# SiftScience/kafka-assigner

Measured on NVIDIA H100. Metric: partition-replica assignments/sec, higher is better.
Workload: dtype int32

## Files before the change

### kafka_assigner_b200/csrc/kassign.cu

```cuda
#include "kassign_stage.cuh"
#include "kassign_order.cuh"
#include "kassign_json.cuh"
#include "kassign_score.cuh"
#include "kassign_waves.cuh"
#include "kassign_waves_json.cuh"
#include "kassign_usage.cuh"

#include <algorithm>
#include <climits>
#include <cmath>
#include <cstdio>
#include <cstdlib>
#include <cstring>
#include <map>
#include <new>
#include <string>
#include <unordered_map>
#include <vector>

#include "../../include/kassign.h"

namespace {

constexpr int KA_SM_COUNT_FALLBACK = 132;
constexpr size_t KA_SMEM_BUDGET = 200 * 1024;
constexpr uint32_t KA_LUT_SMEM_MAX_RANGE = 32768;
constexpr uint32_t KA_LUT_GLOBAL_MAX_RANGE = 1u << 25;

struct DevBuf {
    void* p = nullptr;
    size_t cap = 0;
    cudaError_t reserve(size_t bytes) {
        if (bytes <= cap) return cudaSuccess;
        if (p) cudaFree(p);
        p = nullptr;
        cap = 0;
        size_t want = bytes + bytes / 8 + 256;
        cudaError_t e = cudaMalloc(&p, want);
        if (e == cudaSuccess) cap = want;
        return e;
    }
    void release() {
        if (p) cudaFree(p);
        p = nullptr;
        cap = 0;
    }
    template <typename T> T* as() const { return reinterpret_cast<T*>(p); }
};

constexpr int KA_MAX_BLOCKS = 8;
constexpr int KA_MAX_CHAIN_BLOCKS = 16;
constexpr int KA_MAX_CHAIN_EVENTS = KA_MAX_BLOCKS * KA_MAX_CHAIN_BLOCKS;
constexpr int KA_MAX_JSON_FRAGS = 256;
constexpr int KA_MAX_CANDIDATES = 128;
static_assert(KA_MAX_CANDIDATES <= KA_JSON_MAX_SEGS, "a fleet's documents are built in one segmented JSON pass");
constexpr int64_t KA_JSON_FRAG_ROWS = 1 << 18;

struct HostPinned {
    int err_topic;
    int spin_flag;
    int4 tstatus;
};

struct Plan {
    int a_blob_bytes;
    int a_warps, a_load_bytes, a_slab_bytes, a_cnt_bytes, a_load_kind;
    int a_levels;
    int lv_owner_bytes, lv_last_bytes, lv_p_bytes;
    size_t a_smem;
    int rec_kind, rec_bytes;
    int b_gctr;
    int b_ring_log2;
    int b_threads;
    size_t b_smem;
};

struct StageDesc {
    int topic_base = 0, T = 0;
    int64_t Q = 0;
    const int32_t* d_hash = nullptr;
    const int64_t* d_part_off = nullptr;
    const int64_t* d_rep_off = nullptr;
    int P = 0, RF = 0;
    const int32_t* d_cur = nullptr;
    int desired_rf = -1, S = 1, Pmax = 0;
    int64_t capmax = 0;
    int64_t q0 = 0;
    int blk = 0;
    Plan pl;
};

struct RunScratch {
    DevBuf rec, perm, ntl, lend, loff, lvl_end, tstatus, flags;
    cudaError_t reserve(size_t rec_bytes, size_t q, size_t T, size_t nloff, bool levels, size_t nflags) {
        const struct { DevBuf* b; size_t bytes; } want[] = {
            {&rec, rec_bytes}, {&perm, levels ? q * 2 : 0}, {&lend, levels ? q * 4 : 0}, {&lvl_end, levels ? q * 4 : 0},
            {&ntl, levels ? T * 4 : 0}, {&loff, levels ? nloff * 4 : 0}, {&tstatus, T * sizeof(int4)}, {&flags, nflags * 4},
        };
        for (const auto& w : want)
            if (cudaError_t e = w.b->reserve(w.bytes)) return e;
        return cudaSuccess;
    }
    void release() {
        for (DevBuf* b : {&rec, &perm, &ntl, &lend, &loff, &lvl_end, &tstatus, &flags}) b->release();
    }
};

}

struct ka_ctx {
    int device = 0;
    int sm_count = KA_SM_COUNT_FALLBACK;
    cudaStream_t stream = nullptr;
    cudaStream_t aux = nullptr;
    cudaStream_t sb1 = nullptr;
    cudaStream_t sj = nullptr;
    KaBrokers br{};
    std::vector<int32_t> broker_id;
    DevBuf d_blob, d_glut, d_broker_id, d_ctr8;
    std::unordered_map<int32_t, std::vector<int32_t>> parked;
    int64_t launches = 0;
    DevBuf d_hash, d_part_off, d_rep_off, d_cur, d_out, d_out_len;
    RunScratch run;
    DevBuf d_json, d_names, d_name_off, d_part_id, d_json_rowlen, d_json_blocksum, d_json_state;
    DevBuf d_json_seg;
    DevBuf d_batch_tab, d_batch_ctr;
    RunScratch batch_run;
    DevBuf d_score_w, d_score_sum, d_score_brk, d_score_off;
    DevBuf d_wv_nrecv, d_wv_wave, d_wv_tmp, d_wv_rec, d_wv_cnt, d_wv_state, d_wv_log, d_wv_sum, d_wv_meta;
    DevBuf d_wv_send, d_wv_slog, d_wv_ssum;
    DevBuf d_wv_perm, d_wv_hist, d_wv_doc;
    DevBuf d_wv_part, d_wv_jump;
    DevBuf d_wv_back, d_wv_bscr;
    DevBuf d_us_id, d_us_base, d_us_cap, d_us_before, d_us_ev, d_us_hist, d_us_out, d_us_meta;
    HostPinned* h_pin = nullptr;
    unsigned long long* h_frag = nullptr;
    cudaEvent_t ev[6] = {};
    cudaEvent_t ev_pipe[KA_MAX_BLOCKS][5] = {};
    cudaEvent_t ev_chain[KA_MAX_BLOCKS][4] = {};
    cudaEvent_t ev_in = nullptr, ev_stage[KA_MAX_BLOCKS] = {}, ev_chain_in = nullptr, ev_b1[KA_MAX_CHAIN_EVENTS] = {};
    cudaEvent_t ev_b2[KA_MAX_CHAIN_EVENTS] = {}, ev_emit_done = nullptr;
    cudaEvent_t ev_json_in[KA_MAX_JSON_FRAGS] = {}, ev_json_scan[KA_MAX_JSON_FRAGS] = {}, ev_out_done = nullptr;
    bool timing = false;
    float last_ms[8] = {};
    bool ev_valid = false;
    int last_stages = 1;
    int chain_used = 0;
    bool slot_timed[2] = {false, false};
    int32_t order_plan[8] = {};
    int32_t stage_plan[8] = {};
    bool staged = false;
    StageDesc staged_block;
    int topic_base = 0;
    bool last_was_staged = false;
    cudaStream_t last_stream = nullptr;
    bool pending_status = false;
    ka_status last{};
};

namespace {

#define KA_CUDA(call)                                                                              \
    do {                                                                                           \
        cudaError_t _e = (call);                                                                   \
        if (_e != cudaSuccess) {                                                                   \
            std::fprintf(stderr, "[kassign] CUDA error %s at %s:%d: %s\n", cudaGetErrorName(_e), __FILE__, __LINE__, \
                         cudaGetErrorString(_e));                                                  \
            return KA_ERR_CUDA;                                                                    \
        }                                                                                          \
    } while (0)

int set_status(ka_status* st, int code, int topic = -1, int part = -1, int a = 0, int b = 0) {
    if (st) {
        st->code = code;
        st->topic_index = topic;
        st->partition = part;
        st->a = a;
        st->b = b;
    }
    return code;
}

int failed(ka_status* st, int rc) {
    if (st && st->code != rc) set_status(st, rc);
    return rc;
}

inline size_t align16(size_t v) { return (v + 15) & ~size_t(15); }

template <typename F>
void for_each_event(ka_ctx* c, F f) {
    const struct { cudaEvent_t* e; size_t n; bool timed; } pools[] = {
        {c->ev, sizeof(c->ev) / sizeof(cudaEvent_t), true},
        {&c->ev_pipe[0][0], sizeof(c->ev_pipe) / sizeof(cudaEvent_t), true},
        {&c->ev_chain[0][0], sizeof(c->ev_chain) / sizeof(cudaEvent_t), true},
        {&c->ev_in, 1, false},
        {c->ev_stage, KA_MAX_BLOCKS, false},
        {&c->ev_chain_in, 1, false},
        {c->ev_b1, KA_MAX_CHAIN_EVENTS, false},
        {c->ev_b2, KA_MAX_CHAIN_EVENTS, false},
        {&c->ev_emit_done, 1, false},
        {c->ev_json_in, KA_MAX_JSON_FRAGS, false},
        {c->ev_json_scan, KA_MAX_JSON_FRAGS, false},
        {&c->ev_out_done, 1, false},
    };
    for (const auto& p : pools)
        for (size_t i = 0; i < p.n; ++i) f(p.e[i], p.timed);
}

int park_counters(ka_ctx* c) {
    if (c->br.N == 0 || !c->d_ctr8.p) return KA_OK;
    std::vector<int32_t> h((size_t)c->br.N * KA_MAX_SLOTS);
    KA_CUDA(cudaMemcpy(h.data(), c->d_ctr8.p, h.size() * 4, cudaMemcpyDeviceToHost));
    for (int i = 0; i < c->br.N; ++i) {
        const int32_t* row = h.data() + (size_t)i * KA_MAX_SLOTS;
        bool nz = false;
        for (int r = 0; r < KA_MAX_SLOTS; ++r) nz |= row[r] != 0;
        if (nz) c->parked[c->broker_id[i]] = std::vector<int32_t>(row, row + KA_MAX_SLOTS);
        else c->parked.erase(c->broker_id[i]);
    }
    return KA_OK;
}

int check_brokers(int N, const int32_t* broker_id, const int32_t* broker_rack) {
    if (N < 0 || (N > 0 && (!broker_id || !broker_rack))) return KA_ERR_BAD_ARG;
    if (N > 65535) return KA_ERR_LIMIT;
    for (int i = 0; i < N; ++i) {
        if (i > 0 && broker_id[i] <= broker_id[i - 1]) return KA_ERR_BAD_ARG;
        if (broker_rack[i] < 0 || broker_rack[i] >= 65535) return KA_ERR_BAD_ARG;
    }
    return KA_OK;
}

struct BrokerTable {
    int lut_mode = KA_LUT_SMEM, min_id = 0, lut_off = 0;
    uint32_t range = 0;
    std::vector<uint16_t> blob, glut;
    int blob_bytes() const { return (int)(blob.size() * 2); }
    KaBrokers device(int N, const uint16_t* d_blob, const uint16_t* d_glut, const int32_t* d_broker_id) const {
        return KaBrokers{N, lut_mode, lut_off, blob_bytes(), min_id, range, d_blob, d_glut, d_broker_id};
    }
};

BrokerTable broker_table(int N, const int32_t* broker_id, const int32_t* broker_rack) {
    BrokerTable t;
    t.min_id = N > 0 ? broker_id[0] : 0;
    const uint64_t range64 = N > 0 ? (uint64_t)((int64_t)broker_id[N - 1] - (int64_t)broker_id[0]) + 1 : 0;
    const size_t npad = align16((size_t)std::max(N, 1) * 2) / 2;
    std::vector<uint16_t> rackc(std::max(N, 1), 0);
    {
// ... 121 lines not shown
    d.T = t1 - t0;
    d.blk = blk;
    d.q0 = (int64_t)t0 * sh.P;
    d.Q = ragged ? sh.Q : (int64_t)d.T * sh.P;
    d.d_hash = sh.d_hash + t0;
    d.d_part_off = sh.d_part_off;
    d.d_rep_off = sh.d_rep_off;
    d.P = sh.P;
    d.RF = sh.RF;
    d.d_cur = sh.d_cur + d.q0 * sh.RF;
    d.desired_rf = sh.desired_rf;
    d.S = sh.S;
    d.Pmax = sh.Pmax;
    d.capmax = sh.capmax;
    return make_plan(N, blob_bytes, d.Q, d.S, d.Pmax, d.capmax, ragged, d.pl, st);
}

int reserve_scratch(ka_ctx* c, const StageDesc* ds, int K) {
    const StageDesc& e = ds[K - 1];
    const size_t q = (size_t)std::max<int64_t>(e.q0 + e.Q, 1);
    const size_t T = (size_t)std::max(e.topic_base + e.T, 1);
    KA_CUDA(c->run.reserve(q * ds[0].pl.rec_bytes + 256, q, T, T + K + 1, ds[0].pl.a_levels, 16));
    return KA_OK;
}

int reserve_io(ka_ctx* c, Shape& sh, bool ragged) {
    KA_CUDA(c->d_hash.reserve((size_t)std::max(sh.T, 1) * 4));
    if (ragged) {
        KA_CUDA(c->d_part_off.reserve((size_t)(sh.T + 1) * 8));
        KA_CUDA(c->d_rep_off.reserve((size_t)(sh.Q + 1) * 8));
    }
    KA_CUDA(c->d_cur.reserve((size_t)std::max<int64_t>(sh.R, 1) * 4));
    KA_CUDA(c->d_out.reserve((size_t)std::max<int64_t>(sh.Q, 1) * sh.S * 4));
    KA_CUDA(c->d_out_len.reserve((size_t)std::max<int64_t>(sh.Q, 1) * 4));
    sh.d_hash = c->d_hash.as<int32_t>();
    sh.d_cur = c->d_cur.as<int32_t>();
    if (ragged) {
        sh.d_part_off = c->d_part_off.as<int64_t>();
        sh.d_rep_off = c->d_rep_off.as<int64_t>();
    }
    return KA_OK;
}

int reset_flags(ka_ctx* c, cudaStream_t s) {
    c->h_pin->err_topic = -1;
    c->h_pin->spin_flag = -1;
    c->chain_used = 0;
    c->slot_timed[0] = c->slot_timed[1] = false;
    KA_CUDA(cudaMemsetAsync(c->run.flags.p, 0xFF, 2 * sizeof(int), s));
    return KA_OK;
}

template <typename LoadT, bool LEVELS, int SM, bool CAND>
cudaError_t launch_stage_t(ka_ctx* c, cudaStream_t s, const KaSolveParams& p, const Plan& pl, int T, int ncand, int* grid_x) {
    auto kern = ka_sticky_spread_kernel<LoadT, LEVELS, SM, CAND>;
    const int threads = pl.a_warps * 32;
    cudaError_t e = allow_smem(kern, pl.a_smem);
    if (e != cudaSuccess) return e;
    int occ = 1;
    e = cudaOccupancyMaxActiveBlocksPerMultiprocessor(&occ, kern, threads, pl.a_smem);
    if (e != cudaSuccess) return e;
    int grid = (T + pl.a_warps - 1) / pl.a_warps;
    grid = std::min(grid, std::max(1, std::max(1, occ) * c->sm_count / std::max(ncand, 1)));
    *grid_x = grid;
    kern<<<dim3(grid, std::max(ncand, 1)), threads, pl.a_smem, s>>>(p, pl.a_load_bytes, pl.a_slab_bytes, pl.a_cnt_bytes, pl.lv_owner_bytes,
                                                                 pl.lv_last_bytes, pl.lv_p_bytes);
    return cudaGetLastError();
}

template <typename LoadT, bool LEVELS, bool CAND>
cudaError_t launch_stage(ka_ctx* c, cudaStream_t s, const KaSolveParams& p, const Plan& pl, int T, int ncand, int* grid_x) {
    return p.S <= 3 ? launch_stage_t<LoadT, LEVELS, 3, CAND>(c, s, p, pl, T, ncand, grid_x)
                    : launch_stage_t<LoadT, LEVELS, 8, CAND>(c, s, p, pl, T, ncand, grid_x);
}

void reset_plans(ka_ctx* c) {
    for (int32_t& v : c->order_plan) v = 0;
    for (int32_t& v : c->stage_plan) v = 0;
}

template <bool CAND>
int launch_stage_plan(ka_ctx* c, cudaStream_t s, const KaSolveParams& p, const Plan& pl, int T, int ncand, int lut_mask) {
    cudaError_t e;
    int grid_x = 0;
    if (!pl.a_levels) e = launch_stage<uint8_t, false, CAND>(c, s, p, pl, T, ncand, &grid_x);
    else if (pl.a_load_kind == 0) e = launch_stage<uint8_t, true, CAND>(c, s, p, pl, T, ncand, &grid_x);
    else e = launch_stage<uint16_t, true, CAND>(c, s, p, pl, T, ncand, &grid_x);
    KA_CUDA(e);
    c->launches++;
    int32_t* r = c->stage_plan;
    r[0] = pl.a_load_kind == 0 ? 1 : 2;
    r[1] = pl.a_levels;
    r[2] = p.S <= 3 ? 3 : 8;
    r[3] = ncand;
    r[4] = pl.a_warps;
    r[5] = grid_x;
    r[6] = lut_mask;
    r[7]++;
    return KA_OK;
}

KaSolveParams stage_params(const StageDesc& d) {
    KaSolveParams p{};
    p.T = d.T;
    p.topic_base = d.topic_base;
    p.topic_hash = d.d_hash;
    p.part_off = d.d_part_off;
    p.P = d.P;
    p.rep_off = d.d_rep_off;
    p.RF = d.RF;
    p.cur = d.d_cur;
    p.desired_rf = d.desired_rf;
    p.S = d.S;
    p.Pmax = d.Pmax;
    p.blob_space = d.pl.a_blob_bytes;
    p.rec_kind = d.pl.rec_kind;
    p.chunk_w = d.pl.b_threads;
    return p;
}

int enq_stage(ka_ctx* c, cudaStream_t s, const StageDesc& d, cudaEvent_t a_done, cudaEvent_t done = nullptr) {
    const Plan& pl = d.pl;
    RunScratch& r = c->run;
    if (d.T > 0) {
        KaSolveParams p = stage_params(d);
        p.br = c->br;
        p.out.rec = r.rec.as<unsigned char>() + (size_t)d.q0 * pl.rec_bytes;
        p.out.perm = pl.a_levels ? r.perm.as<uint16_t>() + d.q0 : nullptr;
        p.out.ntl = pl.a_levels ? r.ntl.as<int32_t>() + d.topic_base : nullptr;
        p.out.lend = pl.a_levels ? r.lend.as<uint32_t>() + d.q0 : nullptr;
        p.out.tstatus = r.tstatus.as<int4>();
        p.out.err_topic = r.flags.as<unsigned>();
        const int rc = launch_stage_plan<false>(c, s, p, pl, d.T, 0, 1 << c->br.lut_mode);
        if (rc != KA_OK) return rc;
    }
    const bool tables = pl.a_levels && d.T > 0;
    if (done && !tables) KA_CUDA(cudaEventRecord(done, s));
    if (c->timing) KA_CUDA(cudaEventRecord(a_done, s));
    if (tables) {
        int32_t* ntl = r.ntl.as<int32_t>() + d.topic_base;
        int32_t* loff = r.loff.as<int32_t>() + d.topic_base + d.blk;
        ka_level_scan_kernel<<<1, 1024, 0, s>>>(ntl, d.T, loff);
        KA_CUDA(cudaGetLastError());
        ka_level_fill_kernel<<<(d.T + 7) / 8, 256, 0, s>>>(ntl, loff, r.lend.as<uint32_t>() + d.q0, d.d_part_off, d.P, d.T, d.T, d.Q,
                                                            r.lvl_end.as<uint32_t>() + d.q0);
        KA_CUDA(cudaGetLastError());
        c->launches += 2;
        if (done) KA_CUDA(cudaEventRecord(done, s));
    }
    return KA_OK;
}

template <int KIND, int MAXNT, bool CAND, bool GCTR, bool SINGLE, bool WARP1, bool FULL>
cudaError_t launch_order_t(cudaStream_t s, const KaOrderParams& o, const Plan& pl, int ncand, bool behind) {
    auto kern = ka_order_levels_kernel<KIND, GCTR, MAXNT, SINGLE, WARP1, FULL, CAND>;
    cudaError_t e = allow_smem(kern, pl.b_smem);
    if (e != cudaSuccess) return e;
    cudaLaunchAttribute attr{};
    attr.id = cudaLaunchAttributeProgrammaticStreamSerialization;
    attr.val.programmaticStreamSerializationAllowed = 1;
    cudaLaunchConfig_t cfg{};
    cfg.gridDim = dim3(CAND ? ncand : 1);
    cfg.blockDim = dim3(pl.b_threads);
    cfg.dynamicSmemBytes = pl.b_smem;
    cfg.stream = s;
    cfg.attrs = &attr;
    cfg.numAttrs = behind ? 1 : 0;
    return cudaLaunchKernelEx(&cfg, kern, o);
}

template <int KIND, int MAXNT, bool CAND = false>
cudaError_t launch_order(cudaStream_t s, const KaOrderParams& o, const Plan& pl, int* sel, int ncand = 0, bool behind = false) {
    if constexpr (KIND > 1) {
        *sel = pl.b_gctr ? 4 : 0;
        return pl.b_gctr ? launch_order_t<KIND, MAXNT, false, true, false, false, false>(s, o, pl, ncand, behind)
                         : launch_order_t<KIND, MAXNT, false, false, false, false, false>(s, o, pl, ncand, behind);
    } else {
        const bool warp1 = pl.b_threads == 32;
        const bool single = !warp1 && o.uniform_width != 0 && o.uniform_width <= (uint32_t)pl.b_threads;
        const bool full = single && o.uniform_width == (uint32_t)pl.b_threads;
        *sel = (pl.b_gctr ? 4 : 0) | (warp1 ? 1 : (full ? 3 : (single ? 2 : 0)));
        switch (*sel) {
            case 0: return launch_order_t<KIND, MAXNT, CAND, false, false, false, false>(s, o, pl, ncand, behind);
            case 1: return launch_order_t<KIND, MAXNT, CAND, false, false, true, false>(s, o, pl, ncand, behind);
            case 2: return launch_order_t<KIND, MAXNT, CAND, false, true, false, false>(s, o, pl, ncand, behind);
            case 3: return launch_order_t<KIND, MAXNT, CAND, false, true, false, true>(s, o, pl, ncand, behind);
            case 4: return launch_order_t<KIND, MAXNT, CAND, true, false, false, false>(s, o, pl, ncand, behind);
            case 5: return launch_order_t<KIND, MAXNT, CAND, true, false, true, false>(s, o, pl, ncand, behind);
            case 6: return launch_order_t<KIND, MAXNT, CAND, true, true, false, false>(s, o, pl, ncand, behind);
            default: return launch_order_t<KIND, MAXNT, CAND, true, true, false, true>(s, o, pl, ncand, behind);
        }
    }
}

void note_order(ka_ctx* c, const Plan& pl, int sel, int ncand) {
    int32_t* r = c->order_plan;
    r[0] = pl.rec_kind;
    r[1] = pl.a_levels;
    r[2] = pl.b_threads;
    r[3] = pl.b_ring_log2;
    r[4] = (sel >> 2) & 1;
    r[5] = sel & 3;
    r[6]++;
    r[7] = ncand;
}

constexpr int KA_CHAIN_SUB_TOPICS = 512;
constexpr int KA_CHAIN_LARGE_BLOCK = 1024;

int chain_subblocks(const StageDesc& d, int blocks_in_solve, bool overlapped = false) {
    if (d.d_part_off || d.pl.rec_kind != 3 || d.T < 2) return 1;
    int n = std::max(1, 8 / std::max(1, blocks_in_solve));
    n = std::min(n, std::max(1, d.T / 128));
    if (overlapped && d.T >= KA_CHAIN_LARGE_BLOCK) n = std::max(n, d.T / KA_CHAIN_SUB_TOPICS);
    if (const char* e = std::getenv("KA_CHAIN_SUBBLOCKS")) n = std::max(1, std::min(std::atoi(e), d.T));
    return std::min(n, KA_MAX_CHAIN_BLOCKS);
}

struct SolveCall {
    const int32_t* h_hash = nullptr;
    const int32_t* h_cur = nullptr;
    const int64_t* h_part_off = nullptr;
    const int64_t* h_rep_off = nullptr;
    const int32_t* h_part_id = nullptr;
    int32_t* d_part_id = nullptr;
    int32_t* d_out = nullptr;
    int32_t* d_out_len = nullptr;
    int32_t* h_out = nullptr;
    int32_t* h_out_len = nullptr;
    bool json = false;
    bool stream_out = false;
    int json_blocks = 0;
    int chains = 0;
    bool emits = false;

    SolveCall(int32_t* out, int32_t* out_len) : d_out(out), d_out_len(out_len) {}
};

SolveCall host_call(ka_ctx* c, const int32_t* topic_hash, const int64_t* part_off, const int64_t* rep_off, const int32_t* cur_broker,
                    int32_t* out_len, int32_t* out_broker, const int32_t* part_id = nullptr) {
    SolveCall io(c->d_out.as<int32_t>(), c->d_out_len.as<int32_t>());
    io.h_hash = topic_hash;
    io.h_part_off = part_off;
    io.h_rep_off = rep_off;
    io.h_cur = cur_broker;
    io.h_part_id = part_id;
    io.d_part_id = part_id ? c->d_part_id.as<int32_t>() : nullptr;
    io.h_out = out_broker;
    io.h_out_len = out_len;
    return io;
}

struct SubBlock { int t0, t1; int64_t r0, rq; };

SubBlock sub_block(const StageDesc& d, int j, int nsub) {
    SubBlock b;
    b.t0 = (int)((int64_t)d.T * j / nsub);
    b.t1 = (int)((int64_t)d.T * (j + 1) / nsub);
    b.r0 = d.d_part_off ? 0 : (int64_t)b.t0 * d.P;
    b.rq = d.d_part_off ? d.Q : (int64_t)(b.t1 - b.t0) * d.P;
    return b;
// ... 79 lines not shown
        r += step;
    } while (r < b.rq);
    return KA_OK;
}

int enq_copy_out(cudaStream_t s, const SolveCall& io, int S, int64_t r0, int64_t rows) {
    KA_CUDA(cudaMemcpyAsync(io.h_out + r0 * S, io.d_out + r0 * S, (size_t)rows * S * 4, cudaMemcpyDeviceToHost, s));
    if (io.h_out_len) KA_CUDA(cudaMemcpyAsync(io.h_out_len + r0, io.d_out_len + r0, (size_t)rows * 4, cudaMemcpyDeviceToHost, s));
    return KA_OK;
}

KaOrderParams order_params(ka_ctx* c, const StageDesc& d, const SubBlock& b) {
    const Plan& pl = d.pl;
    KaOrderParams o{};
    o.N = c->br.N;
    o.S = d.S;
    o.uniform_width = pl.a_levels ? 0u : (uint32_t)d.P;
    o.chunk_end = pl.a_levels ? c->run.lvl_end.as<uint32_t>() + d.q0 : nullptr;
    o.ctr8 = c->d_ctr8.as<int32_t>();
    o.ring_log2 = pl.b_ring_log2;
    const int32_t* loff = pl.a_levels ? c->run.loff.as<int32_t>() + d.topic_base + d.blk : nullptr;
    o.Q = (uint32_t)b.rq;
    o.rec = c->run.rec.as<unsigned char>() + (size_t)(d.q0 + b.r0) * pl.rec_bytes;
    o.pos_base = (uint32_t)b.r0;
    o.chunk_lo_ptr = loff ? loff + b.t0 : nullptr;
    o.chunk_hi_ptr = loff ? loff + b.t1 : nullptr;
    return o;
}

int enq_slot_chain(ka_ctx* c, cudaStream_t s, const StageDesc& d, int slot, int j, int nsub, bool behind = false) {
    const SubBlock b = sub_block(d, j, nsub);
    if (b.rq <= 0 || c->br.N <= 0) return KA_OK;
    const KaOrderParams o = order_params(c, d, b);
    int sel = 0;
    KA_CUDA((slot == 0 ? launch_order<0, 1024>(s, o, d.pl, &sel, 0, behind) : launch_order<1, 1024>(s, o, d.pl, &sel, 0, behind)));
    note_order(c, d.pl, sel, 0);
    c->launches++;
    return KA_OK;
}

int enq_emit_block(ka_ctx* c, cudaStream_t s, const StageDesc& d, int j, int nsub, int32_t* d_out, int32_t* d_out_len) {
    const Plan& pl = d.pl;
    const SubBlock b = sub_block(d, j, nsub);
    if (b.rq <= 0 || c->br.N <= 0) return KA_OK;
    ka_emit3_kernel<<<(unsigned)((b.rq + 255) / 256), 256, 0, s>>>(
        reinterpret_cast<const uint4*>(c->run.rec.as<unsigned char>() + (size_t)(d.q0 + b.r0) * pl.rec_bytes),
        pl.a_levels ? c->run.perm.as<uint16_t>() + d.q0 + b.r0 : nullptr, d.d_part_off, b.t1 - b.t0, d.P, c->d_broker_id.as<int32_t>(),
        (uint32_t)b.rq, d.S, d_out + (size_t)b.r0 * d.S, d_out_len ? d_out_len + b.r0 : nullptr, c->d_ctr8.as<int32_t>());
    KA_CUDA(cudaGetLastError());
    c->launches++;
    return KA_OK;
}

int enq_order_emit(ka_ctx* c, cudaStream_t s, const StageDesc& d, SolveCall& io, int blocks_in_solve, cudaEvent_t next_stage = nullptr) {
    const int S = d.S;
    const Plan& pl = d.pl;
    if (next_stage && (d.Q <= 0 || c->br.N <= 0 || pl.rec_kind != 3)) KA_CUDA(cudaStreamWaitEvent(c->sb1, next_stage, 0));
    if (d.Q <= 0 || c->br.N <= 0) return io.json && d.d_part_off && d.Q == 0 ? enq_json(c, s, io, d, sub_block(d, 0, 1), true, true) : KA_OK;
    int32_t* d_out = io.d_out + d.q0 * S;
    int32_t* d_out_len = io.d_out_len ? io.d_out_len + d.q0 : nullptr;
    if (pl.rec_kind != 3) {
        const SubBlock b = sub_block(d, 0, 1);
        KaOrderParams o = order_params(c, d, b);
        o.broker_id = c->d_broker_id.as<int32_t>();
        o.out = d_out;
        o.out_len = d_out_len;
        int sel = 0;
        KA_CUDA((pl.rec_kind == 4 ? launch_order<4, 512>(s, o, pl, &sel) : launch_order<8, 256>(s, o, pl, &sel)));
        note_order(c, pl, sel, 0);
        c->launches++;
        if (io.json) return enq_json(c, s, io, d, b, d.blk == 0, d.blk == blocks_in_solve - 1);
        return KA_OK;
    }
    const int nsub = chain_subblocks(d, blocks_in_solve, true);
    const int e = c->chain_used;
    if (e >= KA_MAX_BLOCKS || io.chains + nsub > KA_MAX_CHAIN_EVENTS) return KA_ERR_LIMIT;
    cudaStream_t s1 = c->sb1, se = c->sj;
    const int jw = nsub > 1 ? nsub - 1 : nsub;
    if (c->timing && e == 0) KA_CUDA(cudaEventRecord(c->ev_chain[0][0], s1));
    for (int j = 0; j < nsub; ++j) {
        const int k = io.chains + j;
        if (next_stage && j == jw) KA_CUDA(cudaStreamWaitEvent(s1, next_stage, 0));
        int rc = enq_slot_chain(c, s1, d, 0, j, nsub, true);
        if (rc != KA_OK) return rc;
        KA_CUDA(cudaEventRecord(c->ev_b1[k], s1));
        KA_CUDA(cudaStreamWaitEvent(s, c->ev_b1[k], 0));
        if (c->timing && j == 0 && e == 0) KA_CUDA(cudaEventRecord(c->ev_chain[0][2], s));
        if ((rc = enq_slot_chain(c, s, d, 1, j, nsub, true)) != KA_OK) return rc;
        KA_CUDA(cudaEventRecord(c->ev_b2[k], s));
        KA_CUDA(cudaStreamWaitEvent(se, c->ev_b2[k], 0));
        if ((rc = enq_emit_block(c, se, d, j, nsub, d_out, d_out_len)) != KA_OK) return rc;
        if (j == nsub - 1) {
            if (c->timing) KA_CUDA(cudaEventRecord(c->ev_chain[0][3], se));
            KA_CUDA(cudaEventRecord(c->ev_emit_done, se));
            io.emits = true;
        }
        const SubBlock b = sub_block(d, j, nsub);
        if (io.stream_out && (rc = enq_copy_out(se, io, S, d.q0 + b.r0, b.rq)) != KA_OK) return rc;
        if (io.json && (rc = enq_json(c, se, io, d, b, d.blk == 0 && j == 0, d.blk == blocks_in_solve - 1 && j == nsub - 1)) != KA_OK)
            return rc;
    }
    if (next_stage && jw == nsub) KA_CUDA(cudaStreamWaitEvent(s1, next_stage, 0));
    if (c->timing && !next_stage) KA_CUDA(cudaEventRecord(c->ev_chain[0][1], s1));
    io.chains += nsub;
    c->chain_used = e + 1;
    return KA_OK;
}

int join_emits(ka_ctx* c, cudaStream_t s, const SolveCall& io) {
    if (io.emits) KA_CUDA(cudaStreamWaitEvent(s, c->ev_emit_done, 0));
    return KA_OK;
}

int chain_fork(ka_ctx* c, cudaStream_t s) {
    KA_CUDA(cudaEventRecord(c->ev_chain_in, s));
    KA_CUDA(cudaStreamWaitEvent(c->sb1, c->ev_chain_in, 0));
    return KA_OK;
}

int enq_solve_end(ka_ctx* c, cudaStream_t s) {
    KA_CUDA(cudaMemcpyAsync(&c->h_pin->err_topic, c->run.flags.p, 2 * sizeof(int), cudaMemcpyDeviceToHost, s));
    if (c->timing) {
        KA_CUDA(cudaEventRecord(c->ev[5], s));
        c->ev_valid = true;
    }
    return KA_OK;
}

int pipeline_stages(int T, int64_t Q) {
    int k = Q >= 262144 ? std::min(4, T / 2048) : 1;
    if (const char* e = std::getenv("KA_PIPELINE_STAGES")) k = std::atoi(e);
    return std::max(1, std::min(k, std::min(KA_MAX_BLOCKS, std::max(T, 1))));
}

int enq_inputs(cudaStream_t s, const SolveCall& io, const StageDesc& d, int64_t ncur) {
    auto h2d = [&](const void* dst, const void* src, size_t bytes) {
        return cudaMemcpyAsync(const_cast<void*>(dst), src, bytes, cudaMemcpyHostToDevice, s);
    };
    if (io.h_hash && d.T > 0) KA_CUDA(h2d(d.d_hash, io.h_hash + d.topic_base, (size_t)d.T * 4));
    if (io.h_part_off && d.T > 0) KA_CUDA(h2d(d.d_part_off, io.h_part_off, (size_t)(d.T + 1) * 8));
    if (io.h_rep_off && d.Q > 0) KA_CUDA(h2d(d.d_rep_off, io.h_rep_off, (size_t)(d.Q + 1) * 8));
    if (io.h_part_id && d.Q > 0) KA_CUDA(h2d(io.d_part_id, io.h_part_id, (size_t)d.Q * 4));
    if (io.h_cur && ncur > 0) KA_CUDA(h2d(d.d_cur, io.h_cur + d.q0 * d.RF, (size_t)ncur * 4));
    return KA_OK;
}

int run_solve(ka_ctx* c, cudaStream_t s, const Shape& sh, SolveCall& io, ka_status* st) {
    c->staged = false;
    c->last_was_staged = false;
    reset_plans(c);
    const bool ragged = sh.d_part_off != nullptr;
    const int T = sh.T;
    const int K = ragged ? 1 : pipeline_stages(T, (int64_t)T * sh.P);
    const bool host_io = (io.h_cur != nullptr || io.h_out != nullptr) && K >= 3;
    const int wsum = host_io ? 2 * (K - 1) : K;
    auto bound = [&](int k) { return k <= 0 ? 0 : (k >= K ? T : (int)((int64_t)T * (host_io ? 2 * k - 1 : k) / wsum)); };
    StageDesc ds[KA_MAX_BLOCKS];
    int rc;
    for (int k = 0; k < K; ++k)
        if ((rc = describe_block(sh, bound(k), bound(k + 1), k, c->br.N, c->br.blob_bytes, ds[k], st)) != KA_OK) return rc;
    if ((rc = reserve_scratch(c, ds, K)) != KA_OK) return rc;
    c->last_stages = K;
    if (c->timing) KA_CUDA(cudaEventRecord(c->ev[0], s));
    if (K == 1) {
        const StageDesc& d = ds[0];
        if ((rc = enq_inputs(s, io, d, ragged ? sh.R : d.Q * d.RF)) != KA_OK) return rc;
        if ((rc = reset_flags(c, s)) != KA_OK) return rc;
        if (c->timing) KA_CUDA(cudaEventRecord(c->ev[1], s));
        if ((rc = enq_stage(c, s, d, c->ev[2])) != KA_OK) return rc;
        if (c->timing) KA_CUDA(cudaEventRecord(c->ev[3], s));
        if ((rc = chain_fork(c, s)) != KA_OK) return rc;
        if ((rc = enq_order_emit(c, s, d, io, 1)) != KA_OK || (rc = join_emits(c, s, io)) != KA_OK) return rc;
        if (c->timing) KA_CUDA(cudaEventRecord(c->ev[4], s));
        if (io.h_out && d.Q > 0 && c->br.N > 0 && (rc = enq_copy_out(s, io, d.S, 0, d.Q)) != KA_OK) return rc;
    } else {
        cudaStream_t aux = c->aux;
        io.stream_out = io.h_out && ds[0].pl.rec_kind == 3 && !io.json;
        KA_CUDA(cudaEventRecord(c->ev_in, s));
        if (io.stream_out) KA_CUDA(cudaStreamWaitEvent(c->sj, c->ev_in, 0));
        KA_CUDA(cudaStreamWaitEvent(aux, c->ev_in, 0));
        if ((rc = reset_flags(c, aux)) != KA_OK) return rc;
        for (int k = 0; k < K; ++k) {
            const StageDesc& d = ds[k];
            if ((rc = enq_inputs(aux, io, d, d.Q * d.RF)) != KA_OK) return rc;
            if (c->timing) KA_CUDA(cudaEventRecord(c->ev_pipe[k][0], aux));
            if ((rc = enq_stage(c, aux, d, c->ev_pipe[k][1], c->ev_stage[k])) != KA_OK) return rc;
            if (c->timing) KA_CUDA(cudaEventRecord(c->ev_pipe[k][2], aux));
        }
        for (int k = 0; k < K; ++k) {
            const StageDesc& d = ds[k];
            KA_CUDA(cudaStreamWaitEvent(s, c->ev_stage[k], 0));
            if (k == 0) {
                KA_CUDA(cudaStreamWaitEvent(c->sb1, c->ev_stage[0], 0));
                KA_CUDA(cudaStreamWaitEvent(c->sb1, c->ev_in, 0));
            }
            if (c->timing && k == 0) KA_CUDA(cudaEventRecord(c->ev_pipe[0][3], s));
            if ((rc = enq_order_emit(c, s, d, io, K, k + 1 < K ? c->ev_stage[k + 1] : nullptr)) != KA_OK) return rc;
            if (c->timing && k == K - 1) KA_CUDA(cudaEventRecord(c->ev_pipe[K - 1][4], s));
            if (io.h_out && !io.stream_out && d.Q > 0 && c->br.N > 0 && (rc = enq_copy_out(s, io, d.S, d.q0, d.Q)) != KA_OK) return rc;
        }
        if ((rc = join_emits(c, s, io)) != KA_OK) return rc;
        if (io.stream_out) {
            KA_CUDA(cudaEventRecord(c->ev_out_done, c->sj));
            KA_CUDA(cudaStreamWaitEvent(s, c->ev_out_done, 0));
        }
    }
    return enq_solve_end(c, s);
}

ka_status topic_status(int t, const int4& ts, const int32_t* part_id, const int64_t* part_off) {
    ka_status r;
    set_status(&r, ts.x, t, ts.y >= 0 && part_id && part_off ? part_id[part_off[t] + ts.y] : ts.y, ts.z, ts.w);
    return r;
}

int finish_status(ka_ctx* c, cudaStream_t s, ka_status* st, const int32_t* part_id = nullptr, const int64_t* part_off = nullptr) {
    KA_CUDA(cudaStreamSynchronize(s));
    c->pending_status = false;
    ka_status r{};
    set_status(&r, KA_OK);
    if (c->h_pin->err_topic != -1) {
        const int t = c->h_pin->err_topic;
        KA_CUDA(cudaMemcpy(&c->h_pin->tstatus, c->run.tstatus.as<int4>() + t, sizeof(int4), cudaMemcpyDeviceToHost));
        r = topic_status(t, c->h_pin->tstatus, part_id, part_off);
        r.topic_index += c->last_was_staged ? c->topic_base : 0;
    }
    if (c->timing && c->ev_valid) {
        for (int i = 0; i < 8; ++i) c->last_ms[i] = 0.f;
        cudaEventElapsedTime(&c->last_ms[5], c->ev[0], c->ev[5]);
        if (c->last_stages <= 1) {
            cudaEventElapsedTime(&c->last_ms[3], c->ev[0], c->ev[1]);
            cudaEventElapsedTime(&c->last_ms[0], c->ev[1], c->ev[2]);
            cudaEventElapsedTime(&c->last_ms[1], c->ev[2], c->ev[3]);
            cudaEventElapsedTime(&c->last_ms[7], c->ev[3], c->ev[4]);
            cudaEventElapsedTime(&c->last_ms[4], c->ev[4], c->ev[5]);
        } else {
            for (int k = 0; k < c->last_stages; ++k) {
                float a = 0.f, t = 0.f;
                cudaEventElapsedTime(&a, c->ev_pipe[k][0], c->ev_pipe[k][1]);
                cudaEventElapsedTime(&t, c->ev_pipe[k][1], c->ev_pipe[k][2]);
                c->last_ms[0] += a;
                c->last_ms[1] += t;
            }
            cudaEventElapsedTime(&c->last_ms[7], c->ev_pipe[0][3], c->ev_pipe[c->last_stages - 1][4]);
        }
        if (c->chain_used > 0) {
            cudaEventElapsedTime(&c->last_ms[2], c->ev_chain[0][0], c->ev_chain[0][1]);
            cudaEventElapsedTime(&c->last_ms[6], c->ev_chain[0][2], c->ev_chain[0][3]);
        } else if (c->slot_timed[0] || c->slot_timed[1]) {
            if (c->slot_timed[0]) cudaEventElapsedTime(&c->last_ms[2], c->ev_chain[0][0], c->ev_chain[0][1]);
            if (c->slot_timed[1]) cudaEventElapsedTime(&c->last_ms[6], c->ev_chain[1][0], c->ev_chain[1][1]);
        } else {
            c->last_ms[2] = c->last_ms[7];
        }
    }
    c->last = r;
    if (st) *st = r;
    return r.code;
}

int enter(ka_ctx* c, bool collect) {
    KA_CUDA(cudaSetDevice(c->device));
    if (collect && c->pending_status) finish_status(c, c->last_stream, nullptr);
    return KA_OK;
}

int finish(ka_ctx* c, cudaStream_t s, ka_status* st, bool sync, const int32_t* part_id = nullptr, const int64_t* part_off = nullptr) {
    c->last_stream = s;
    c->pending_status = true;
    return st || sync ? finish_status(c, s, st, part_id, part_off) : KA_OK;
}

int fail_members(ka_status* st, int K, int rc) {
    for (int k = 0; k < K; ++k) set_status(st + k, rc);
    return rc;
}

int abort_batch(ka_ctx* c, cudaStream_t s, ka_status* st, int K, int rc) {
    cudaStreamSynchronize(c->sb1);
    cudaStreamSynchronize(s);
    return fail_members(st, K, rc);
}

int batch_args(ka_ctx* c, int K, int out_stride, ka_status* st) {
    if (!st || K < 0) return KA_ERR_BAD_ARG;
    for (int k = 0; k < K; ++k) set_status(st + k, KA_OK);
    if (!c) return fail_members(st, K, KA_ERR_NO_DEVICE);
    if (K > KA_MAX_CANDIDATES || out_stride > 3) return fail_members(st, K, KA_ERR_LIMIT);
    if (out_stride < 1) return fail_members(st, K, KA_ERR_BAD_ARG);
    return KA_OK;
}

// ... 127 lines not shown
}

extern "C" {

const char* ka_version(void) { return "kassign-b200 0.1 (sm_90a)"; }

int32_t ka_java_string_hash(const char* s) {
    uint32_t h = 0;
    const unsigned char* u = reinterpret_cast<const unsigned char*>(s);
    while (*u) {
        uint32_t cp;
        int extra;
        unsigned char b = *u++;
        if (b < 0x80) { cp = b; extra = 0; }
        else if ((b & 0xE0) == 0xC0) { cp = b & 0x1F; extra = 1; }
        else if ((b & 0xF0) == 0xE0) { cp = b & 0x0F; extra = 2; }
        else if ((b & 0xF8) == 0xF0) { cp = b & 0x07; extra = 3; }
        else { cp = 0xFFFD; extra = 0; }
        while (extra-- > 0 && *u) cp = (cp << 6) | (*u++ & 0x3F);
        if (cp >= 0x10000) {
            cp -= 0x10000;
            h = h * 31u + (0xD800u + (cp >> 10));
            h = h * 31u + (0xDC00u + (cp & 0x3FFu));
        } else {
            h = h * 31u + cp;
        }
    }
    return (int32_t)h;
}

int32_t ka_rack_indices(int32_t N, const int32_t* broker_id, const char* const* rack_name, int32_t* broker_rack) {
    if (N < 0 || (N > 0 && (!broker_id || !broker_rack))) return KA_ERR_BAD_ARG;
    std::map<std::string, int32_t> key2idx;
    for (int i = 0; i < N; ++i) {
        std::string key = (rack_name && rack_name[i]) ? std::string(rack_name[i]) : std::to_string(broker_id[i]);
        auto it = key2idx.find(key);
        if (it == key2idx.end()) it = key2idx.emplace(key, (int32_t)key2idx.size()).first;
        broker_rack[i] = it->second;
    }
    return KA_OK;
}

ka_ctx* ka_ctx_create(int32_t device) {
    int ndev = 0;
    if (cudaGetDeviceCount(&ndev) != cudaSuccess || ndev <= 0 || device < 0 || device >= ndev) {
        cudaGetLastError();
        return nullptr;
    }
    if (cudaSetDevice(device) != cudaSuccess) return nullptr;
    ka_ctx* c = new (std::nothrow) ka_ctx();
    if (!c) return nullptr;
    c->device = device;
    cudaDeviceProp prop;
    if (cudaGetDeviceProperties(&prop, device) == cudaSuccess) c->sm_count = prop.multiProcessorCount;
    bool ok = cudaHostAlloc(reinterpret_cast<void**>(&c->h_pin), sizeof(HostPinned), cudaHostAllocDefault) == cudaSuccess &&
              cudaHostAlloc(reinterpret_cast<void**>(&c->h_frag), 2 * KA_MAX_JSON_FRAGS * sizeof(unsigned long long),
                            cudaHostAllocDefault) == cudaSuccess;
    for (cudaStream_t* s : {&c->stream, &c->aux, &c->sb1, &c->sj})
        ok = ok && cudaStreamCreateWithFlags(s, cudaStreamNonBlocking) == cudaSuccess;
    for_each_event(c, [&](cudaEvent_t& e, bool timed) {
        ok = ok && cudaEventCreateWithFlags(&e, timed ? cudaEventDefault : cudaEventDisableTiming) == cudaSuccess;
    });
    if (!ok) {
        ka_ctx_destroy(c);
        return nullptr;
    }
    return c;
}

void ka_ctx_destroy(ka_ctx* c) {
    if (!c) return;
    cudaSetDevice(c->device);
    for (cudaStream_t s : {c->stream, c->aux, c->sb1, c->sj})
        if (s) cudaStreamSynchronize(s);
    for (DevBuf* b : {&c->d_blob, &c->d_glut, &c->d_broker_id, &c->d_ctr8, &c->d_hash, &c->d_part_off, &c->d_rep_off, &c->d_cur,
                      &c->d_out, &c->d_out_len, &c->d_json, &c->d_names, &c->d_name_off, &c->d_part_id, &c->d_json_rowlen,
                      &c->d_json_blocksum, &c->d_json_state, &c->d_batch_tab, &c->d_batch_ctr, &c->d_score_w, &c->d_score_sum,
                      &c->d_score_brk, &c->d_score_off, &c->d_json_seg, &c->d_wv_nrecv, &c->d_wv_wave, &c->d_wv_tmp, &c->d_wv_rec,
                      &c->d_wv_cnt, &c->d_wv_state, &c->d_wv_log, &c->d_wv_sum, &c->d_wv_meta, &c->d_wv_perm, &c->d_wv_hist, &c->d_wv_doc,
                      &c->d_wv_part, &c->d_wv_jump, &c->d_wv_send, &c->d_wv_slog, &c->d_wv_ssum, &c->d_us_id, &c->d_us_base,
                      &c->d_us_cap, &c->d_us_before, &c->d_us_ev, &c->d_us_hist, &c->d_us_out, &c->d_us_meta})
        b->release();
    c->run.release();
    c->batch_run.release();
    for_each_event(c, [](cudaEvent_t& e, bool) {
        if (e) cudaEventDestroy(e);
    });
    for (cudaStream_t s : {c->stream, c->aux, c->sb1, c->sj})
        if (s) cudaStreamDestroy(s);
    if (c->h_pin) cudaFreeHost(c->h_pin);
    if (c->h_frag) cudaFreeHost(c->h_frag);
    delete c;
}

int32_t ka_ctx_reset(ka_ctx* c) {
    if (!c) return KA_ERR_NO_DEVICE;
    int rc = enter(c, true);
    if (rc != KA_OK) return rc;
    c->parked.clear();
    if (c->br.N > 0 && c->d_ctr8.p) KA_CUDA(cudaMemset(c->d_ctr8.p, 0, (size_t)c->br.N * KA_MAX_SLOTS * 4));
    return KA_OK;
}

int32_t ka_ctx_set_brokers(ka_ctx* c, int32_t N, const int32_t* broker_id, const int32_t* broker_rack) {
    if (!c) return KA_ERR_NO_DEVICE;
    int rc = check_brokers(N, broker_id, broker_rack);
    if (rc != KA_OK) return rc;
// ... 1556 lines not shown
```

Before: 3.230 billion.

## Split first stage into head block and reserve SMs for overlapping chain

In the multi-stage path, the first block's stage kernel is split into a small head sub-block, launched with fewer warps, and a remaining part. This lets the order/emit chain for the first sub-block start earlier while the rest of the stage runs. The stage kernels are also padded in shared memory and given a smaller grid so that a few SMs stay free for the concurrent chain kernels. Later stages are enqueued lazily, interleaved with the chain. The cost is extra launches and less stage parallelism, and the shared-memory padding used to keep SMs free depends on device properties.

Result: faster. 3.339 billion (median of 6 runs) (+3.3%).

```diff
diff --git a/kafka_assigner_b200/csrc/kassign.cu b/kafka_assigner_b200/csrc/kassign.cu
--- a/kafka_assigner_b200/csrc/kassign.cu
+++ b/kafka_assigner_b200/csrc/kassign.cu
@@ -7,6 +7,7 @@
 #include "kassign_usage.cuh"
 
 #include <algorithm>
+#include <functional>
 #include <climits>
 #include <cmath>
 #include <cstdio>
@@ -111,6 +112,7 @@
 struct ka_ctx {
     int device = 0;
     int sm_count = KA_SM_COUNT_FALLBACK;
+    size_t smem_per_sm = 0, smem_reserved = 0;
     cudaStream_t stream = nullptr;
     cudaStream_t aux = nullptr;
     cudaStream_t sb1 = nullptr;
@@ -138,13 +140,15 @@
     cudaEvent_t ev[6] = {};
     cudaEvent_t ev_pipe[KA_MAX_BLOCKS][5] = {};
     cudaEvent_t ev_chain[KA_MAX_BLOCKS][4] = {};
-    cudaEvent_t ev_in = nullptr, ev_stage[KA_MAX_BLOCKS] = {}, ev_chain_in = nullptr, ev_b1[KA_MAX_CHAIN_EVENTS] = {};
+    cudaEvent_t ev_head_t[2] = {};
+    cudaEvent_t ev_in = nullptr, ev_stage[KA_MAX_BLOCKS] = {}, ev_head = nullptr, ev_chain_in = nullptr, ev_b1[KA_MAX_CHAIN_EVENTS] = {};
     cudaEvent_t ev_b2[KA_MAX_CHAIN_EVENTS] = {}, ev_emit_done = nullptr;
     cudaEvent_t ev_json_in[KA_MAX_JSON_FRAGS] = {}, ev_json_scan[KA_MAX_JSON_FRAGS] = {}, ev_out_done = nullptr;
     bool timing = false;
     float last_ms[8] = {};
     bool ev_valid = false;
     int last_stages = 1;
+    bool last_head_split = false;
     int chain_used = 0;
     bool slot_timed[2] = {false, false};
     int32_t order_plan[8] = {};
@@ -194,8 +198,10 @@
         {c->ev, sizeof(c->ev) / sizeof(cudaEvent_t), true},
         {&c->ev_pipe[0][0], sizeof(c->ev_pipe) / sizeof(cudaEvent_t), true},
         {&c->ev_chain[0][0], sizeof(c->ev_chain) / sizeof(cudaEvent_t), true},
+        {c->ev_head_t, 2, true},
         {&c->ev_in, 1, false},
         {c->ev_stage, KA_MAX_BLOCKS, false},
+        {&c->ev_head, 1, false},
         {&c->ev_chain_in, 1, false},
         {c->ev_b1, KA_MAX_CHAIN_EVENTS, false},
         {c->ev_b2, KA_MAX_CHAIN_EVENTS, false},
@@ -423,26 +429,31 @@
 }
 
 template <typename LoadT, bool LEVELS, int SM, bool CAND>
-cudaError_t launch_stage_t(ka_ctx* c, cudaStream_t s, const KaSolveParams& p, const Plan& pl, int T, int ncand, int* grid_x) {
+cudaError_t launch_stage_t(ka_ctx* c, cudaStream_t s, const KaSolveParams& p, const Plan& pl, int T, int ncand, int keep_free, int* grid_x) {
     auto kern = ka_sticky_spread_kernel<LoadT, LEVELS, SM, CAND>;
     const int threads = pl.a_warps * 32;
-    cudaError_t e = allow_smem(kern, pl.a_smem);
+    int64_t smem = (int64_t)pl.a_smem;
+    if (keep_free > 0) {
+        const int64_t per_sm = (int64_t)c->smem_per_sm, rsv = (int64_t)c->smem_reserved;
+        smem = std::max({smem, per_sm / 2 - rsv + 1, per_sm - 2 * rsv - (int64_t)pl.b_smem + 1});
+    }
+    cudaError_t e = allow_smem(kern, (size_t)smem);
     if (e != cudaSuccess) return e;
     int occ = 1;
-    e = cudaOccupancyMaxActiveBlocksPerMultiprocessor(&occ, kern, threads, pl.a_smem);
+    e = cudaOccupancyMaxActiveBlocksPerMultiprocessor(&occ, kern, threads, (size_t)smem);
     if (e != cudaSuccess) return e;
     int grid = (T + pl.a_warps - 1) / pl.a_warps;
-    grid = std::min(grid, std::max(1, std::max(1, occ) * c->sm_count / std::max(ncand, 1)));
+    grid = std::min(grid, std::max(1, std::max(1, occ) * (c->sm_count - keep_free) / std::max(ncand, 1)));
     *grid_x = grid;
-    kern<<<dim3(grid, std::max(ncand, 1)), threads, pl.a_smem, s>>>(p, pl.a_load_bytes, pl.a_slab_bytes, pl.a_cnt_bytes, pl.lv_owner_bytes,
-                                                                 pl.lv_last_bytes, pl.lv_p_bytes);
+    kern<<<dim3(grid, std::max(ncand, 1)), threads, (size_t)smem, s>>>(p, pl.a_load_bytes, pl.a_slab_bytes, pl.a_cnt_bytes,
+                                                                       pl.lv_owner_bytes, pl.lv_last_bytes, pl.lv_p_bytes);
     return cudaGetLastError();
 }
 
 template <typename LoadT, bool LEVELS, bool CAND>
-cudaError_t launch_stage(ka_ctx* c, cudaStream_t s, const KaSolveParams& p, const Plan& pl, int T, int ncand, int* grid_x) {
-    return p.S <= 3 ? launch_stage_t<LoadT, LEVELS, 3, CAND>(c, s, p, pl, T, ncand, grid_x)
-                    : launch_stage_t<LoadT, LEVELS, 8, CAND>(c, s, p, pl, T, ncand, grid_x);
+cudaError_t launch_stage(ka_ctx* c, cudaStream_t s, const KaSolveParams& p, const Plan& pl, int T, int ncand, int keep_free, int* grid_x) {
+    return p.S <= 3 ? launch_stage_t<LoadT, LEVELS, 3, CAND>(c, s, p, pl, T, ncand, keep_free, grid_x)
+                    : launch_stage_t<LoadT, LEVELS, 8, CAND>(c, s, p, pl, T, ncand, keep_free, grid_x);
 }
 
 void reset_plans(ka_ctx* c) {
@@ -451,12 +462,12 @@
 }
 
 template <bool CAND>
-int launch_stage_plan(ka_ctx* c, cudaStream_t s, const KaSolveParams& p, const Plan& pl, int T, int ncand, int lut_mask) {
+int launch_stage_plan(ka_ctx* c, cudaStream_t s, const KaSolveParams& p, const Plan& pl, int T, int ncand, int lut_mask, int keep_free = 0) {
     cudaError_t e;
     int grid_x = 0;
-    if (!pl.a_levels) e = launch_stage<uint8_t, false, CAND>(c, s, p, pl, T, ncand, &grid_x);
-    else if (pl.a_load_kind == 0) e = launch_stage<uint8_t, true, CAND>(c, s, p, pl, T, ncand, &grid_x);
-    else e = launch_stage<uint16_t, true, CAND>(c, s, p, pl, T, ncand, &grid_x);
+    if (!pl.a_levels) e = launch_stage<uint8_t, false, CAND>(c, s, p, pl, T, ncand, keep_free, &grid_x);
+    else if (pl.a_load_kind == 0) e = launch_stage<uint8_t, true, CAND>(c, s, p, pl, T, ncand, keep_free, &grid_x);
+    else e = launch_stage<uint16_t, true, CAND>(c, s, p, pl, T, ncand, keep_free, &grid_x);
     KA_CUDA(e);
     c->launches++;
     int32_t* r = c->stage_plan;
@@ -490,7 +501,7 @@
     return p;
 }
 
-int enq_stage(ka_ctx* c, cudaStream_t s, const StageDesc& d, cudaEvent_t a_done, cudaEvent_t done = nullptr) {
+int enq_stage(ka_ctx* c, cudaStream_t s, const StageDesc& d, cudaEvent_t a_done, cudaEvent_t done = nullptr, int keep_free = 0) {
     const Plan& pl = d.pl;
     RunScratch& r = c->run;
     if (d.T > 0) {
@@ -502,7 +513,7 @@
         p.out.lend = pl.a_levels ? r.lend.as<uint32_t>() + d.q0 : nullptr;
         p.out.tstatus = r.tstatus.as<int4>();
         p.out.err_topic = r.flags.as<unsigned>();
-        const int rc = launch_stage_plan<false>(c, s, p, pl, d.T, 0, 1 << c->br.lut_mode);
+        const int rc = launch_stage_plan<false>(c, s, p, pl, d.T, 0, 1 << c->br.lut_mode, keep_free);
         if (rc != KA_OK) return rc;
     }
     const bool tables = pl.a_levels && d.T > 0;
@@ -578,6 +589,7 @@
 
 constexpr int KA_CHAIN_SUB_TOPICS = 512;
 constexpr int KA_CHAIN_LARGE_BLOCK = 1024;
+constexpr int KA_CHAIN_SMS = 4;
 
 int chain_subblocks(const StageDesc& d, int blocks_in_solve, bool overlapped = false) {
     if (d.d_part_off || d.pl.rec_kind != 3 || d.T < 2) return 1;
@@ -763,10 +775,17 @@
     return KA_OK;
 }
 
-int enq_order_emit(ka_ctx* c, cudaStream_t s, const StageDesc& d, SolveCall& io, int blocks_in_solve, cudaEvent_t next_stage = nullptr) {
+int enq_order_emit(ka_ctx* c, cudaStream_t s, const StageDesc& d, SolveCall& io, int blocks_in_solve, cudaEvent_t next_stage = nullptr,
+                   cudaEvent_t rest_stage = nullptr, const std::function<int()>* enq_next = nullptr) {
     const int S = d.S;
     const Plan& pl = d.pl;
-    if (next_stage && (d.Q <= 0 || c->br.N <= 0 || pl.rec_kind != 3)) KA_CUDA(cudaStreamWaitEvent(c->sb1, next_stage, 0));
+    auto wait_next = [&]() -> int {
+        const int r = enq_next ? (*enq_next)() : KA_OK;
+        if (r == KA_OK) KA_CUDA(cudaStreamWaitEvent(c->sb1, next_stage, 0));
+        return r;
+    };
+    int rc;
+    if (next_stage && (d.Q <= 0 || c->br.N <= 0 || pl.rec_kind != 3) && (rc = wait_next()) != KA_OK) return rc;
     if (d.Q <= 0 || c->br.N <= 0) return io.json && d.d_part_off && d.Q == 0 ? enq_json(c, s, io, d, sub_block(d, 0, 1), true, true) : KA_OK;
     int32_t* d_out = io.d_out + d.q0 * S;
     int32_t* d_out_len = io.d_out_len ? io.d_out_len + d.q0 : nullptr;
@@ -791,8 +810,10 @@
     if (c->timing && e == 0) KA_CUDA(cudaEventRecord(c->ev_chain[0][0], s1));
     for (int j = 0; j < nsub; ++j) {
         const int k = io.chains + j;
-        if (next_stage && j == jw) KA_CUDA(cudaStreamWaitEvent(s1, next_stage, 0));
-        int rc = enq_slot_chain(c, s1, d, 0, j, nsub, true);
+        if (enq_next && j == 1 && (rc = (*enq_next)()) != KA_OK) return rc;
+        if (rest_stage && j == 1) KA_CUDA(cudaStreamWaitEvent(s1, rest_stage, 0));
+        if (next_stage && j == jw && (rc = wait_next()) != KA_OK) return rc;
+        rc = enq_slot_chain(c, s1, d, 0, j, nsub, true);
         if (rc != KA_OK) return rc;
         KA_CUDA(cudaEventRecord(c->ev_b1[k], s1));
         KA_CUDA(cudaStreamWaitEvent(s, c->ev_b1[k], 0));
@@ -811,7 +832,7 @@
         if (io.json && (rc = enq_json(c, se, io, d, b, d.blk == 0 && j == 0, d.blk == blocks_in_solve - 1 && j == nsub - 1)) != KA_OK)
             return rc;
     }
-    if (next_stage && jw == nsub) KA_CUDA(cudaStreamWaitEvent(s1, next_stage, 0));
+    if (next_stage && jw == nsub && (rc = wait_next()) != KA_OK) return rc;
     if (c->timing && !next_stage) KA_CUDA(cudaEventRecord(c->ev_chain[0][1], s1));
     io.chains += nsub;
     c->chain_used = e + 1;
@@ -872,6 +893,7 @@
         if ((rc = describe_block(sh, bound(k), bound(k + 1), k, c->br.N, c->br.blob_bytes, ds[k], st)) != KA_OK) return rc;
     if ((rc = reserve_scratch(c, ds, K)) != KA_OK) return rc;
     c->last_stages = K;
+    c->last_head_split = false;
     if (c->timing) KA_CUDA(cudaEventRecord(c->ev[0], s));
     if (K == 1) {
         const StageDesc& d = ds[0];
@@ -891,22 +913,58 @@
         if (io.stream_out) KA_CUDA(cudaStreamWaitEvent(c->sj, c->ev_in, 0));
         KA_CUDA(cudaStreamWaitEvent(aux, c->ev_in, 0));
         if ((rc = reset_flags(c, aux)) != KA_OK) return rc;
+        const bool split = !io.h_cur && ds[0].pl.rec_kind == 3 && !ds[0].pl.a_levels && ds[0].T >= KA_CHAIN_LARGE_BLOCK &&
+                           chain_subblocks(ds[0], K, true) >= 2;
+        const int keep_free = split ? KA_CHAIN_SMS : 0;
+        c->last_head_split = split;
+        StageDesc head, rest;
+        if (split) {
+            const int t1 = sub_block(ds[0], 0, chain_subblocks(ds[0], K, true)).t1;
+            if ((rc = describe_block(sh, 0, t1, 0, c->br.N, c->br.blob_bytes, head, st)) != KA_OK ||
+                (rc = describe_block(sh, t1, bound(1), 0, c->br.N, c->br.blob_bytes, rest, st)) != KA_OK)
+                return rc;
+            Plan& hp = head.pl;
+            const int sms = std::max(1, c->sm_count - keep_free);
+            const int w = std::max(1, std::min(hp.a_warps, (head.T + sms - 1) / sms));
+            hp.a_smem -= (hp.a_smem - 16 - (size_t)hp.a_blob_bytes) / hp.a_warps * (size_t)(hp.a_warps - w);
+            hp.a_warps = w;
+        }
+        auto enq_part = [&](const StageDesc& d, cudaEvent_t start, cudaEvent_t a_done, cudaEvent_t done) -> int {
+            const int r = enq_inputs(aux, io, d, d.Q * d.RF);
+            if (r != KA_OK) return r;
+            if (c->timing) KA_CUDA(cudaEventRecord(start, aux));
+            return enq_stage(c, aux, d, a_done, done, keep_free);
+        };
+        auto stage = [&](int k) -> int {
+            const int r = k == 0 && split ? enq_part(rest, c->ev_head_t[1], c->ev_pipe[0][1], c->ev_stage[0])
+                                          : enq_part(ds[k], c->ev_pipe[k][0], c->ev_pipe[k][1], c->ev_stage[k]);
+            if (r == KA_OK && c->timing) KA_CUDA(cudaEventRecord(c->ev_pipe[k][2], aux));
+            return r;
+        };
+        int staged_k = 0;
+        auto stage_to = [&](int last) -> int {
+            for (; staged_k <= last && staged_k < K; ++staged_k) {
+                const int r = stage(staged_k);
+                if (r != KA_OK) return r;
+            }
+            return KA_OK;
+        };
+        if (split && (rc = enq_part(head, c->ev_pipe[0][0], c->ev_head_t[0], c->ev_head)) != KA_OK) return rc;
+        if ((rc = stage_to(split ? 0 : K - 1)) != KA_OK) return rc;
         for (int k = 0; k < K; ++k) {
             const StageDesc& d = ds[k];
-            if ((rc = enq_inputs(aux, io, d, d.Q * d.RF)) != KA_OK) return rc;
-            if (c->timing) KA_CUDA(cudaEventRecord(c->ev_pipe[k][0], aux));
-            if ((rc = enq_stage(c, aux, d, c->ev_pipe[k][1], c->ev_stage[k])) != KA_OK) return rc;
-            if (c->timing) KA_CUDA(cudaEventRecord(c->ev_pipe[k][2], aux));
-        }
-        for (int k = 0; k < K; ++k) {
-            const StageDesc& d = ds[k];
-            KA_CUDA(cudaStreamWaitEvent(s, c->ev_stage[k], 0));
+            const cudaEvent_t staged = k == 0 && split ? c->ev_head : c->ev_stage[k];
+            KA_CUDA(cudaStreamWaitEvent(s, staged, 0));
             if (k == 0) {
-                KA_CUDA(cudaStreamWaitEvent(c->sb1, c->ev_stage[0], 0));
+                KA_CUDA(cudaStreamWaitEvent(c->sb1, staged, 0));
                 KA_CUDA(cudaStreamWaitEvent(c->sb1, c->ev_in, 0));
             }
             if (c->timing && k == 0) KA_CUDA(cudaEventRecord(c->ev_pipe[0][3], s));
-            if ((rc = enq_order_emit(c, s, d, io, K, k + 1 < K ? c->ev_stage[k + 1] : nullptr)) != KA_OK) return rc;
+            const std::function<int()> enq_next = [&] { return stage_to(k + 1); };
+            if ((rc = enq_order_emit(c, s, d, io, K, k + 1 < K ? c->ev_stage[k + 1] : nullptr,
+                                     k == 0 && split ? c->ev_stage[0] : nullptr, split ? &enq_next : nullptr)) != KA_OK ||
+                (rc = stage_to(k + 1)) != KA_OK)
+                return rc;
             if (c->timing && k == K - 1) KA_CUDA(cudaEventRecord(c->ev_pipe[K - 1][4], s));
             if (io.h_out && !io.stream_out && d.Q > 0 && c->br.N > 0 && (rc = enq_copy_out(s, io, d.S, d.q0, d.Q)) != KA_OK) return rc;
         }
@@ -948,7 +1006,14 @@
         } else {
             for (int k = 0; k < c->last_stages; ++k) {
                 float a = 0.f, t = 0.f;
-                cudaEventElapsedTime(&a, c->ev_pipe[k][0], c->ev_pipe[k][1]);
+                if (k == 0 && c->last_head_split) {
+                    float b = 0.f;
+                    cudaEventElapsedTime(&a, c->ev_pipe[0][0], c->ev_head_t[0]);
+                    cudaEventElapsedTime(&b, c->ev_head_t[1], c->ev_pipe[0][1]);
+                    a += b;
+                } else {
+                    cudaEventElapsedTime(&a, c->ev_pipe[k][0], c->ev_pipe[k][1]);
+                }
                 cudaEventElapsedTime(&t, c->ev_pipe[k][1], c->ev_pipe[k][2]);
                 c->last_ms[0] += a;
                 c->last_ms[1] += t;
@@ -1182,7 +1247,11 @@
     if (!c) return nullptr;
     c->device = device;
     cudaDeviceProp prop;
-    if (cudaGetDeviceProperties(&prop, device) == cudaSuccess) c->sm_count = prop.multiProcessorCount;
+    if (cudaGetDeviceProperties(&prop, device) == cudaSuccess) {
+        c->sm_count = prop.multiProcessorCount;
+        c->smem_per_sm = prop.sharedMemPerMultiprocessor;
+        c->smem_reserved = prop.reservedSharedMemPerBlock;
+    }
     bool ok = cudaHostAlloc(reinterpret_cast<void**>(&c->h_pin), sizeof(HostPinned), cudaHostAllocDefault) == cudaSuccess &&
               cudaHostAlloc(reinterpret_cast<void**>(&c->h_frag), 2 * KA_MAX_JSON_FRAGS * sizeof(unsigned long long),
                             cudaHostAllocDefault) == cudaSuccess;
```
